# LimHaeryong/ESKF_LIO

Hardware: AMD Instinct MI355X
Metric: registered points/sec per VGICP iteration (100k-pt scan vs 1M-voxel map), 1/2/4/8 GPU (higher is better)
Workload: dtype f64

## Files before the change

### eskf_lio_amd/csrc/vgicp_kernels.hip

```cpp
#include <array>
#include <utility>

#include "vgicp_device.h"
#include "vgicp_device_fn.h"
#include "vgicp_launch_plan.h"
#include "vgicp_points_plan.h"

namespace vgicp {
namespace {

template <typename Args>
__device__ __forceinline__ bool scan_cov_symmetric(const Args& a) {
  return a.asym_dev != nullptr && *a.asym_dev != a.scan_seq;
}

template <int PIECES = 1>
__device__ __forceinline__ void unpack_payload(const double2* pay, double (&mu)[3], double (&S)[9]) {
  const double2 a0 = pay[0 * PIECES], a1 = pay[1 * PIECES], a2 = pay[2 * PIECES],
                a3 = pay[3 * PIECES], a4 = pay[4 * PIECES], a5 = pay[5 * PIECES];
  mu[0] = a0.x; mu[1] = a0.y; mu[2] = a1.x;
  S[0] = a1.y; S[1] = a2.x; S[2] = a2.y; S[3] = a3.x; S[4] = a3.y; S[5] = a4.x;
  S[6] = a4.y; S[7] = a5.x; S[8] = a5.y;
}
__device__ __forceinline__ void load_payload(const VoxelRecord* rec, double (&mu)[3], double (&S)[9]) {
// ... 836 lines not shown
  const int c_matched = __syncthreads_count(matched ? 1 : 0);
  const int c_counted = __syncthreads_count(counted ? 1 : 0);
  const int c_negative = __syncthreads_count(negative ? 1 : 0);
  const int c_not_finite = __syncthreads_count(not_finite ? 1 : 0);
  if (threadIdx.x == 0) {
    if (c_matched) atomicAdd(&a.counters[0], (uint32_t)c_matched);
    if (c_counted) atomicAdd(&a.counters[1], (uint32_t)c_counted);
    if (c_negative) atomicAdd(&a.counters[2], (uint32_t)c_negative);
    if (c_not_finite) atomicAdd(&a.counters[3], (uint32_t)c_not_finite);
  }
}

__global__ __launch_bounds__(256) void gate_decide_kernel(GateArgs a) {
  const uint32_t i = blockIdx.x * 256u + threadIdx.x;
  const bool cov_sym = scan_cov_symmetric(a);
  bool matched = false, refused = false, not_finite = false;
  if (i < a.n) {
    const PointTerm term = point_term(a, i, cov_sym);
    matched = term.matched;
    if (matched) {
      not_finite = !(fabs(term.raw) < __builtin_inf());
      refused = not_finite || !(fmax(term.raw, 0.0) <= a.gate);
    }
    a.keep[i] = refused ? (uint8_t)0 : (uint8_t)1;
  }
  const int c_matched = __syncthreads_count(matched ? 1 : 0);
  const int c_refused = __syncthreads_count(refused ? 1 : 0);
  const int c_not_finite = __syncthreads_count(not_finite ? 1 : 0);
  if (threadIdx.x == 0) {
    if (c_matched) atomicAdd(&a.counters[0], (uint32_t)c_matched);
    if (c_refused) atomicAdd(&a.counters[1], (uint32_t)c_refused);
    if (c_not_finite) atomicAdd(&a.counters[2], (uint32_t)c_not_finite);
  }
}

__global__ __launch_bounds__(64) void point_pick_kernel(PointPickArgs a) {
  const uint32_t lane = threadIdx.x;
  if (lane < (uint32_t)kPointCounters) a.out[lane] = a.counters[lane];
  if (lane < a.n_quantiles && lane < (uint32_t)kPointQuantiles) {
    const uint32_t matched = a.counters[0], not_finite = a.counters[3];
    const uint64_t m = matched > not_finite ? matched - not_finite : 0u;
    unsigned long long bits = 0x7FF8000000000000ull;
    if (m > 0) {
      const uint64_t rank = quantile_rank(a.q[lane], m);
      if (rank < a.n) bits = a.sorted[rank];
    }
    a.out[kPointCounters + lane] = bits;
  }
}

__global__ __launch_bounds__(64) void solve_step_kernel(const double* __restrict__ packed, double cos_thr,
                                                        double tsq_thr, int force_pivoted,
                                                        double* __restrict__ out) {
  __shared__ double totals[kSlots];
  __shared__ double work[kSolveWork];
  const uint32_t lane = threadIdx.x;
  if (lane < kSlots) totals[lane] = lane < kNormalEq ? packed[lane] : 0.0;
  __syncthreads();
  double A[21], g[6], xi[6];
#pragma unroll
  for (int k = 0; k < 21; ++k) A[k] = packed[k];
#pragma unroll
  for (int k = 0; k < 6; ++k) g[k] = -packed[21 + k];
  bool pivoted = force_pivoted != 0;
  if (pivoted || !ldlt6_solve_spd(A, g, xi)) {
    ldlt6_solve_pivoted(totals, work, lane, xi);
    pivoted = true;
  }
  Pose step;
  se3_exp_device(xi, step);
  const bool conv = converged(step, cos_thr, tsq_thr);
  if (lane == 0) {
#pragma unroll
    for (int k = 0; k < 6; ++k) out[k] = xi[k];
#pragma unroll
    for (int k = 0; k < 9; ++k) out[6 + k] = step.R[k];
#pragma unroll
    for (int k = 0; k < 3; ++k) out[15 + k] = step.t[k];
    out[18] = pivoted ? 1.0 : 0.0;
    out[19] = conv ? 1.0 : 0.0;
  }
}

typedef __attribute__((address_space(1))) unsigned long long gu64;
typedef __attribute__((address_space(1))) unsigned int gu32;

__device__ __forceinline__ void store_through_bits(double* p, unsigned long long bits) {
  __hip_atomic_store((gu64*)p, bits, __ATOMIC_RELAXED, __HIP_MEMORY_SCOPE_AGENT);
}
__device__ __forceinline__ unsigned long long load_through_bits(const double* p) {
  return __hip_atomic_load((gu64*)p, __ATOMIC_RELAXED, __HIP_MEMORY_SCOPE_AGENT);
}
__device__ __forceinline__ void store_system_bits(double* p, unsigned long long bits) {
  __hip_atomic_store((gu64*)p, bits, __ATOMIC_RELAXED, __HIP_MEMORY_SCOPE_SYSTEM);
}
__device__ __forceinline__ unsigned long long load_system_bits(const double* p) {
  return __hip_atomic_load((gu64*)p, __ATOMIC_RELAXED, __HIP_MEMORY_SCOPE_SYSTEM);
}
__device__ __forceinline__ unsigned long long publishable(double v) {
  const unsigned long long b = (unsigned long long)__double_as_longlong(v);
  return b == kRowUnset ? kRowNaN : b;
}

constexpr int kL2Delay = 64;
template <bool SYSTEM, bool LIVE = false>
__device__ __forceinline__ bool poll_and_sum(const double* src, uint32_t lane, uint32_t spin_limit, double& sum,
                                             uint32_t live = (uint32_t)kFolders) {
  constexpr int H = kFolders / 2;
  const uint32_t slot = lane & 31u, half = lane >> 5;
  const bool active = slot <= (uint32_t)kCountSlot;
  const double* mine = src + (size_t)half * H * kSlots + (active ? slot : 0u);
  unsigned long long w[H];
  if constexpr (LIVE) {
#pragma unroll
    for (int k = 0; k < H; ++k)
      w[k] = (active && half * H + (uint32_t)k < live) ? load_through_bits(mine + k * kSlots) : 0ull;
  } else {
#pragma unroll
    for (int k = 0; k < H; ++k)
      w[k] = active ? (SYSTEM ? load_system_bits(mine + k * kSlots) : load_through_bits(mine + k * kSlots)) : 0ull;
  }
  for (uint32_t spins = 0;; ++spins) {
    bool missing = false;
#pragma unroll
    for (int k = 0; k < H; ++k) missing = missing || (w[k] == kRowUnset);
    if (!__any(missing)) break;
    if (spins >= spin_limit) return false;
    __builtin_amdgcn_s_sleep(1);
#pragma unroll
    for (int k = 0; k < H; ++k)
      if (w[k] == kRowUnset) w[k] = SYSTEM ? load_system_bits(mine + k * kSlots) : load_through_bits(mine + k * kSlots);
  }
  double x[H];
#pragma unroll
  for (int k = 0; k < H; ++k) x[k] = __longlong_as_double((long long)w[k]);
  const double part = tree_sum<H>(x);
  const unsigned plo = (unsigned)__double2loint(part), phi = (unsigned)__double2hiint(part);
  const auto lo = __builtin_amdgcn_permlane32_swap(plo, plo, false, false);
  const auto hi = __builtin_amdgcn_permlane32_swap(phi, phi, false, false);
  sum = part + __hiloint2double((int)hi[1], (int)lo[1]);
  return true;
}

template <int N>
__device__ __forceinline__ uint64_t pinned_clock(double (&x)[N]) {
#pragma unroll
  for (int k = 0; k < N; ++k) asm volatile("" : "+v"(x[k]));
  const uint64_t t = wall_clock64();
#pragma unroll
  for (int k = 0; k < N; ++k) asm volatile("" : "+v"(x[k]));
  return t;
}

__device__ __forceinline__ bool fused_round0_load(const FusedUpload& f, uint64_t stride, uint32_t n_pts, double* lds,
                                                  double (&q0)[kScanPlanes]) {
  typedef int v4i __attribute__((ext_vector_type(4)));
  constexpr uint32_t B = 512, W = B - 64;
  __shared__ uint32_t ok_sh, form_sh[2];
  const uint32_t tid = threadIdx.x, p0 = blockIdx.x * W;
  const uint32_t cnt = p0 < n_pts ? min(W, n_pts - p0) : 0u;
  if (cnt == 0) return true;
  const uint32_t ua = p0 / f.unit, ub = (p0 + cnt - 1) / f.unit;
  const uint32_t split = min(p0 + cnt, (ua + 1) * f.unit);
  if (tid == 0) {
    uint32_t good = 1;
    for (uint32_t u = ua; u <= ub && good; ++u)
      for (uint32_t spins = 0; __hip_atomic_load(f.flags + 16 * u, __ATOMIC_RELAXED, __HIP_MEMORY_SCOPE_SYSTEM) != f.seq; ++spins) {
        if (spins >= f.spin_limit) { good = 0; break; }
        __builtin_amdgcn_s_sleep(20);
      }
    __atomic_thread_fence(__ATOMIC_ACQUIRE);
    ok_sh = good;
    if (good) {
      form_sh[0] = __hip_atomic_load(f.flags + 16 * ua + 1, __ATOMIC_RELAXED, __HIP_MEMORY_SCOPE_SYSTEM);
      form_sh[1] = __hip_atomic_load(f.flags + 16 * ub + 1, __ATOMIC_RELAXED, __HIP_MEMORY_SCOPE_SYSTEM);
    }
  }
  __syncthreads();
  if (!ok_sh) return false;
  double* lp = lds;
  double* lc = lds + 3 * W;
  double* lq = lds + 12 * W;
  {
    const v4i* sp = reinterpret_cast<const v4i*>(f.apts + (size_t)p0 * 24);
    const uint32_t np = (cnt * 24 + 15) / 16;
    for (uint32_t k = tid; k < np; k += B) reinterpret_cast<v4i*>(lp)[k] = __builtin_nontemporal_load(sp + k);
  }
  for (uint32_t s = 0; s < 2; ++s) {
    const uint32_t s0 = s ? split : p0, s1 = s ? p0 + cnt : split, u = s ? ub : ua;
    if (s0 >= s1) continue;
    if (form_sh[s] == kArenaCompact) {
      const v4i* sc = reinterpret_cast<const v4i*>(f.acov + (size_t)u * f.unit * 72 + (size_t)(s0 - u * f.unit) * 48);
      v4i* dst = reinterpret_cast<v4i*>(lq + 6 * (s0 - p0));
      for (uint32_t k = tid; k < (s1 - s0) * 3; k += B) dst[k] = __builtin_nontemporal_load(sc + k);
    } else {
      const v4i* sc = reinterpret_cast<const v4i*>(f.acov + (size_t)s0 * 72);
      v4i* dst = reinterpret_cast<v4i*>(lc + 9 * (s0 - p0));
      const uint32_t nc = ((s1 - s0) * 72 + 15) / 16;
      for (uint32_t k = tid; k < nc; k += B) dst[k] = __builtin_nontemporal_load(sc + k);
    }
  }
  __syncthreads();
  if (tid < cnt && form_sh[p0 + tid >= split ? 1 : 0] == kArenaCompact) {
    const double* q = lq + 6 * tid;
    const double a0 = q[0], a1 = q[1], a2 = q[2], a3 = q[3], a4 = q[4], a5 = q[5];
    double* c = lc + 9 * tid;
    c[0] = a0; c[1] = a1; c[2] = a2; c[3] = a1; c[4] = a3; c[5] = a4; c[6] = a2; c[7] = a4; c[8] = a5;
  }
  __syncthreads();
  if (tid == 0) atomicMax(f.unit_clock, (unsigned long long)wall_clock64());
  {
    const uint32_t wp = 3 * cnt, wc = 9 * cnt;
    v4i* dp = reinterpret_cast<v4i*>(f.aos_pts + 3 * (size_t)p0);
    v4i* dc = reinterpret_cast<v4i*>(f.aos_cov + 9 * (size_t)p0);
    for (uint32_t k = tid; k < wp / 2; k += B) dp[k] = reinterpret_cast<const v4i*>(lp)[k];
    for (uint32_t k = tid; k < wc / 2; k += B) dc[k] = reinterpret_cast<const v4i*>(lc)[k];
    if (tid == 0 && (cnt & 1u)) {
      f.aos_pts[3 * (size_t)p0 + wp - 1] = lp[wp - 1];
      f.aos_cov[9 * (size_t)p0 + wc - 1] = lc[wc - 1];
    }
  }
  const uint32_t wt = tid - 64u;
  if (tid >= 64u && wt < cnt) {
#pragma unroll
    for (int k = 0; k < 3; ++k) q0[k] = lp[3 * wt + k];
#pragma unroll
    for (int k = 0; k < 9; ++k) q0[3 + k] = lc[9 * wt + k];
    const size_t i = p0 + wt;
#pragma unroll
    for (int k = 0; k < kScanPlanes; ++k) f.soa[k * stride + i] = q0[k];
    const bool same = __double_as_longlong(q0[4]) == __double_as_longlong(q0[6]) &&
                      __double_as_longlong(q0[5]) == __double_as_longlong(q0[9]) &&
                      __double_as_longlong(q0[8]) == __double_as_longlong(q0[10]);
    if (!same) *f.asym = f.seq;
  }
  return true;
}

struct TeamView {
  uint32_t vb = 0;
  uint32_t team_wgs = 0;
  uint32_t folder_rows = 0;
  uint32_t* abort_word = nullptr;
};
template <int BLOCK, bool MULTI, bool STAMPS, bool MANY, bool FUSED = false, bool TEAM = false, bool ROBUST = false,
          bool PRIOR = false>
__device__ __forceinline__ void persistent_body(const PersistArgs& a, const FusedUpload& up, const TeamView& tv = TeamView()) {
  static_assert(!ROBUST || (!MULTI && !STAMPS && !FUSED && !TEAM), "the robust round runs the single-device bodies only");
  static_assert(!PRIOR || (!MULTI && !STAMPS && !FUSED && !TEAM), "the pose prior runs the single-device bodies only");
  static_assert(!FUSED || (!MULTI && !STAMPS && !MANY), "the fused upload serves the single-device one-point-per-thread body");
  static_assert(!TEAM || (!MULTI && !STAMPS && !MANY && !FUSED), "teams run the single-device one-point-per-thread body");
  static_assert(BLOCK / kSlots == kFolders, "the exchange reproduces the fold order of iterate_kernel<512>");
  constexpr int kWaves = BLOCK / 64;
  constexpr int kWorkers = BLOCK - 64;
  __shared__ double red[kWaves][kSlots];
  __shared__ double totals[kSlots];
  __shared__ double work[kSolveWork];
  __shared__ double pose_sh[12];
  __shared__ int stop_sh;
  extern __shared__ __attribute__((aligned(16))) unsigned char dyn_lds[];
  int4* pf_key = reinterpret_cast<int4*>(dyn_lds);
  double2* pf_pay = reinterpret_cast<double2*>(dyn_lds + (size_t)kWorkers * sizeof(int4));
  const bool prefetch = !MANY && a.prefetch_margin > 0.0;

  const uint32_t tid = threadIdx.x, lane = tid & 63, wave = tid >> 6;
  const uint32_t n_pts = a.n_dev ? (*a.n_dev < a.n ? *a.n_dev : a.n) : a.n;
  const bool cov_sym = MANY && scan_cov_symmetric(a);
  const uint32_t grid = gridDim.x, blk = TEAM ? tv.vb : blockIdx.x;
  constexpr uint32_t W = MANY ? (uint32_t)BLOCK : (uint32_t)kWorkers;
  const bool worker = MANY || wave != 0;
  const uint32_t wt = MANY ? tid : tid - 64u;
  uint32_t stride_pts = grid * W, first = worker ? blk * W + wt : n_pts, end_pts = n_pts;
  if constexpr (MANY) {
    const uint32_t units = (n_pts + 63u) / 64u, share = units / grid, extra = units % grid;
    const uint32_t u0 = blk * share + (blk < extra ? blk : extra), u1 = u0 + share + (blk < extra ? 1u : 0u);
    stride_pts = W;
    first = u0 * 64u + wt;
    end_pts = u1 * 64u < n_pts ? u1 * 64u : n_pts;
  }
  const VoxelRecord* pay_base = a.dense ? a.dense : a.table;
  int4* memo = reinterpret_cast<int4*>(dyn_lds);
  double* stash = reinterpret_cast<double*>(dyn_lds + (size_t)a.memo_points * W * sizeof(int4));
  const uint32_t park_planes = cov_sym ? 9u : (uint32_t)kScanPlanes;
  const uint32_t fit = a.stash_bytes / (park_planes * W * (uint32_t)sizeof(double));
  const uint32_t parked = MANY ? (fit < a.stash_points ? fit : a.stash_points) : 0u;
  const bool folder = blk < (uint32_t)kFolders;
  const uint32_t my_row = TEAM ? (blk % kFolders) * tv.folder_rows + blk / kFolders : (blk % kFolders) * kFolders + blk / kFolders;
  const uint32_t buf_rows = TEAM ? (uint32_t)kFolders * tv.folder_rows : (uint32_t)kExchangeRows;
  const uint32_t live_rows = TEAM ? (tv.team_wgs - blk + (uint32_t)kFolders - 1u) / (uint32_t)kFolders : (uint32_t)kFolders;
  const uint32_t live_parts = TEAM ? (tv.team_wgs < (uint32_t)kFolders ? tv.team_wgs : (uint32_t)kFolders) : (uint32_t)kFolders;

  Pose total;
#pragma unroll
  for (int k = 0; k < 9; ++k) total.R[k] = a.pose0[k];
#pragma unroll
  for (int k = 0; k < 3; ++k) total.t[k] = a.pose0[9 + k];
  const double cos_thr = a.cosine_threshold, tsq_thr = a.translation_sq_threshold;
  const int max_it = a.max_iteration;
  const double inv_voxel = 1.0 / a.voxel_size;
  const double same_margin = 0x1p-20 * a.voxel_size;
  RobustSetting robust;
  if constexpr (ROBUST) robust = robust_setting(a.robust.kernel, a.robust.scale2, a.robust.gate);

  double q0[kScanPlanes];
#pragma unroll
  for (int k = 0; k < kScanPlanes; ++k) q0[k] = 0.0;
  const bool have = first < end_pts;
  if constexpr (FUSED) {
    if (!fused_round0_load(up, a.stride, n_pts, reinterpret_cast<double*>(dyn_lds), q0)) {
      if (tid == 0) a.state->abort_seq = a.seq;
      return;
    }
  } else if (have) {
    load_point(a.scan, a.stride, first, q0);
  }

  bool spec = false, hit = false;
  int32_t okx = 0, oky = 0, okz = 0;
  double mu[3] = {0.0, 0.0, 0.0}, Sv[9];
#pragma unroll
  for (int k = 0; k < 9; ++k) Sv[k] = 0.0;

  uint64_t t_mark = STAMPS ? wall_clock64() : 0;
  uint64_t acc_body = 0, acc_l1 = 0, acc_l2 = 0, acc_solve = 0;
  uint64_t fine[4] = {0, 0, 0, 0};
  bool conv_keep = false;
  int it = 0;
  bool gave_up = false;
  for (;;) {
    const double* R = total.R;
    const double* t = total.t;
    if (worker) {
      double v[kSlots];
#pragma unroll
      for (int k = 0; k < kSlots; ++k) v[k] = 0.0;
      if constexpr (!MANY) {
        if (have) {
          double p[3], C[9], S[9];
#pragma unroll
          for (int k = 0; k < 9; ++k) C[k] = q0[3 + k];
          transform_point(R, t, q0[0], q0[1], q0[2], p);
          const int32_t kx = voxel_coord_fast(p[0], a.voxel_size, inv_voxel);
          const int32_t ky = voxel_coord_fast(p[1], a.voxel_size, inv_voxel);
          const int32_t kz = voxel_coord_fast(p[2], a.voxel_size, inv_voxel);
          if (!spec || kx != okx || ky != oky || kz != okz) {
            bool served = false;
            if (spec && prefetch) {
              const int4 m = pf_key[tid - 64];
              if (m.x == kx && m.y == ky && m.z == kz && (uint32_t)m.w != kMemoNone) {
                served = true;
                hit = (uint32_t)m.w != kMemoMiss;
                if (hit) unpack_payload<kWorkers>(pf_pay + (tid - 64), mu, Sv);
              }
            }
            if (!served) hit = find_and_load(a.table, a.mask, kx, ky, kz, mu, Sv);
            okx = kx; oky = ky; okz = kz;
            spec = true;
          }
          if (hit) {
#pragma unroll
            for (int k = 0; k < 9; ++k) S[k] = Sv[k];
            accumulate_match<true, ROBUST>(R, p, C, mu, S, v, robust);
          }
        }
      } else {
        auto one_point = [&](const double (&q)[kScanPlanes], uint32_t e, auto first_of_round) {
          double p[3], C[9], m2[3], S[9];
          transform_point(R, t, q[0], q[1], q[2], p);
          bool got;
          if (e < a.memo_points) {
            int4* mslot = memo + (size_t)e * W + wt;
            const int4 m = *mslot;
            const bool stayed = ((int)(it != 0) & (int)same_voxel_coord(p[0], m.x, a.voxel_size, same_margin) &
                                 (int)same_voxel_coord(p[1], m.y, a.voxel_size, same_margin) &
                                 (int)same_voxel_coord(p[2], m.z, a.voxel_size, same_margin)) != 0;
            if (stayed) {
              got = (uint32_t)m.w != kMemoMiss;
              if (got) load_payload(pay_base + (uint32_t)m.w, m2, S);
            } else {
              const int32_t kx = voxel_coord_fast(p[0], a.voxel_size, inv_voxel);
              const int32_t ky = voxel_coord_fast(p[1], a.voxel_size, inv_voxel);
              const int32_t kz = voxel_coord_fast(p[2], a.voxel_size, inv_voxel);
              if (it != 0 && m.x == kx && m.y == ky && m.z == kz) {
                got = (uint32_t)m.w != kMemoMiss;
                if (got) load_payload(pay_base + (uint32_t)m.w, m2, S);
              } else {
                const VoxelRecord* rec = find_voxel(a.table, a.mask, kx, ky, kz);
                got = rec != nullptr;
                uint32_t where = kMemoMiss;
                if (got) where = a.dense ? reinterpret_cast<const uint32_t*>(&rec->reserved)[1] : (uint32_t)(rec - a.table);
                *mslot = make_int4(kx, ky, kz, (int32_t)where);
                if (got) load_payload(rec, m2, S);
              }
            }
          } else {
            const int32_t kx = voxel_coord_fast(p[0], a.voxel_size, inv_voxel);
            const int32_t ky = voxel_coord_fast(p[1], a.voxel_size, inv_voxel);
            const int32_t kz = voxel_coord_fast(p[2], a.voxel_size, inv_voxel);
            got = find_and_load(a.table, a.mask, kx, ky, kz, m2, S);
          }
          if (got) {
#pragma unroll
            for (int k = 0; k < 9; ++k) C[k] = q[3 + k];
            accumulate_match<decltype(first_of_round)::value, ROBUST>(R, p, C, m2, S, v, robust);
          }
        };
        if (have) one_point(q0, 0u, Flag<true>{});
        uint32_t e = 1;
        for (uint32_t i = first + stride_pts; i < end_pts; i += stride_pts, ++e) {
          double q[kScanPlanes];
          if (e <= parked) {
            double* slot = stash + (size_t)(e - 1) * park_planes * W + wt;
            if (it == 0) {
              load_point_sym(a.scan, a.stride, i, q, cov_sym);
              if (cov_sym) {
                constexpr int kUsed[9] = {0, 1, 2, 3, 4, 5, 7, 8, 11};
#pragma unroll
                for (int j = 0; j < 9; ++j) slot[j * W] = q[kUsed[j]];
              } else {
#pragma unroll
                for (int k = 0; k < kScanPlanes; ++k) slot[k * W] = q[k];
              }
            } else if (cov_sym) {
              constexpr int kUsed[9] = {0, 1, 2, 3, 4, 5, 7, 8, 11};
#pragma unroll
              for (int j = 0; j < 9; ++j) q[kUsed[j]] = slot[j * W];
              q[6] = q[4]; q[9] = q[5]; q[10] = q[8];
            } else {
#pragma unroll
              for (int k = 0; k < kScanPlanes; ++k) q[k] = slot[k * W];
            }
          } else {
            load_point_sym(a.scan, a.stride, i, q, cov_sym);
          }
          one_point(q, e, Flag<false>{});
        }
      }
      wave_fold_to_lds(v, lane, red[wave]);
    }
    __syncthreads();
    if (STAMPS) { const uint64_t n = wall_clock64(); acc_body += n - t_mark; t_mark = n; }

    if (!MANY && worker && prefetch && have) {
      double p[3], rx, ry, rz;
      transform_point(R, t, q0[0], q0[1], q0[2], p);
      (void)voxel_coord_fast(p[0], a.voxel_size, inv_voxel, &rx);
      (void)voxel_coord_fast(p[1], a.voxel_size, inv_voxel, &ry);
      (void)voxel_coord_fast(p[2], a.voxel_size, inv_voxel, &rz);
      const double half = 0.5 * a.voxel_size;
      const double dx = fmin(rx, a.voxel_size - rx), dy = fmin(ry, a.voxel_size - ry), dz = fmin(rz, a.voxel_size - rz);
      int32_t nx = okx, ny = oky, nz = okz;
      double d;
      if (dx <= dy && dx <= dz) { d = dx; nx += rx < half ? -1 : 1; }
      else if (dy <= dz) { d = dy; ny += ry < half ? -1 : 1; }
      else { d = dz; nz += rz < half ? -1 : 1; }
      int4 m = make_int4(nx, ny, nz, (int32_t)kMemoNone);
      if (d < a.prefetch_margin * a.voxel_size) {
        const VoxelRecord* rec = find_voxel(a.table, a.mask, nx, ny, nz);
        m.w = rec ? (int32_t)(uint32_t)(rec - a.table) : (int32_t)kMemoMiss;
        if (rec) {
          const double2* pay = reinterpret_cast<const double2*>(rec->mean);
          double2* dst = pf_pay + (tid - 64);
#pragma unroll
          for (int j = 0; j < 6; ++j) dst[j * kWorkers] = pay[j];
        }
      }
      pf_key[tid - 64] = m;
    }
    if (STAMPS && !MANY && wave != 0) { asm volatile("s_waitcnt vmcnt(0) lgkmcnt(0)" ::: "memory"); const uint64_t n = wall_clock64(); acc_l1 += n - t_mark; t_mark = n; }

    if (wave == 0) {
      uint32_t lane_here = tid & 63;
      asm volatile("" : "+v"(lane_here));
      const uint32_t lane = lane_here;
      const uint32_t buf = (a.round0 + (uint32_t)it) % 3u;
      double* rows = a.rows + (size_t)buf * buf_rows * kSlots;
      double* parts = a.parts + (size_t)buf * kFolders * kSlots;
      asm volatile("s_waitcnt vmcnt(0)" ::: "memory");
      if (lane <= (uint32_t)kCountSlot) {
        double w_sum[kWaves];
#pragma unroll
        for (int w = 0; w < kWaves; ++w) w_sum[w] = red[w][lane];
        const double row_sum = MANY ? tree_sum<kWaves>(w_sum) : tree_sum<kWaves - 1>(w_sum + 1);
        store_through_bits(rows + (size_t)my_row * kSlots + lane, publishable(row_sum));
      }
      bool ok = true;
      const uint32_t spin_limit = (FUSED && it == 0 && up.spin_limit > a.spin_limit) ? up.spin_limit : a.spin_limit;
      if (folder) {
        double part = 0.0;
        if constexpr (TEAM) ok = poll_and_sum<false, true>(rows + (size_t)blk * tv.folder_rows * kSlots, lane, spin_limit, part, live_rows);
        else ok = poll_and_sum<false>(rows + (size_t)blk * kFolders * kSlots, lane, spin_limit, part);
        if (ok && lane <= (uint32_t)kCountSlot) store_through_bits(parts + (size_t)blk * kSlots + lane, publishable(part));
      }
      if (STAMPS) { const uint64_t n = wall_clock64(); acc_l1 += n - t_mark; t_mark = n; }
      double tot = 0.0;
      if (!MULTI) {
        if (!MANY && !folder) __builtin_amdgcn_s_sleep(kL2Delay);
        if constexpr (TEAM) { if (ok) ok = poll_and_sum<false, true>(parts, lane, spin_limit, tot, live_parts); }
        else if (ok) ok = poll_and_sum<false>(parts, lane, spin_limit, tot);
      } else {
        const uint32_t mbuf = (a.mail_round0 + (uint32_t)it) % 3u;
        if (blk == 0) {
          double mine = 0.0;
          if (ok) ok = poll_and_sum<false>(parts, lane, a.spin_limit, mine);
          if (ok && lane <= (uint32_t)kCountSlot) {
            const unsigned long long bits = publishable(mine);
            for (uint32_t r = 0; r < a.world; ++r)
              store_system_bits(a.mail[r] + ((size_t)mbuf * kMaxRanks + a.rank) * kSlots + lane, bits);
          }
        }
        if (ok) ok = poll_and_sum<true>(a.mail[a.rank] + (size_t)mbuf * kMaxRanks * kSlots, lane, a.spin_limit, tot);
      }
      if (STAMPS) { const uint64_t n = wall_clock64(); acc_l2 += n - t_mark; t_mark = n; }
      if (!ok) {
        if (lane == 0) stop_sh = 2;
      } else {
        if (lane < kSlots) totals[lane] = lane <= (uint32_t)kCountSlot ? tot : 0.0;
        __builtin_amdgcn_fence(__ATOMIC_RELEASE, "wavefront");
        __builtin_amdgcn_wave_barrier();
        __builtin_amdgcn_fence(__ATOMIC_ACQUIRE, "wavefront");
        const double* solve = totals;
        if constexpr (PRIOR) solve = prior_solve_totals(a, total, totals, lane);
        double A[21], g[6], xi[6];
#pragma unroll
        for (int k = 0; k < 21; ++k) A[k] = solve[k];
#pragma unroll
        for (int k = 0; k < 6; ++k) g[k] = -solve[21 + k];
        uint64_t f0 = 0, f1 = 0, f2 = 0;
        if (STAMPS) { f0 = pinned_clock(A); fine[0] += f0 - t_mark; }
        if (!ldlt6_solve_spd(A, g, xi)) ldlt6_solve_pivoted(solve, work, lane, xi);
        if (STAMPS) { f1 = pinned_clock(xi); fine[1] += f1 - f0; }
        Pose next, step;
        se3_exp_device(xi, step);
        pose_compose(step, total, next);
        conv_keep = converged(step, cos_thr, tsq_thr);
        if (STAMPS) { f2 = pinned_clock(next.R); fine[2] += f2 - f1; }
        if (lane == 0) {
#pragma unroll
          for (int k = 0; k < 9; ++k) pose_sh[k] = next.R[k];
#pragma unroll
          for (int k = 0; k < 3; ++k) pose_sh[9 + k] = next.t[k];
          stop_sh = (conv_keep || (it + 1 >= max_it)) ? 1 : 0;
        }
        if (STAMPS) fine[3] += wall_clock64() - f2;
      }
    }
    __syncthreads();
    const int stop = stop_sh;
    if (stop == 2) { gave_up = true; break; }
    if (wave == 0) {
      uint32_t lane_here = tid & 63;
      asm volatile("" : "+v"(lane_here));
      const uint32_t rearm = (a.round0 + (uint32_t)it + 2u) % 3u;
      if (lane_here <= (uint32_t)kCountSlot) {
        store_through_bits(a.rows + ((size_t)rearm * buf_rows + my_row) * kSlots + lane_here, kRowUnset);
        if (folder) store_through_bits(a.parts + ((size_t)rearm * kFolders + blk) * kSlots + lane_here, kRowUnset);
      }
      if (MULTI && blk == 0 && lane_here <= (uint32_t)kCountSlot) {
        const uint32_t old = (a.mail_round0 + (uint32_t)it + 2u) % 3u;
        for (uint32_t r = 0; r < a.world; ++r)
          store_system_bits(a.mail[a.rank] + ((size_t)old * kMaxRanks + r) * kSlots + lane_here, kRowUnset);
      }
      if (blk == 0 && lane_here < kSlots) a.log[(size_t)it * kSlots + lane_here] = totals[lane_here];
    }
    load_pose(pose_sh, total);
    ++it;
    if (STAMPS) { const uint64_t n = wall_clock64(); acc_solve += n - t_mark; t_mark = n; }
    if (stop) break;
  }
  if (gave_up) {
    if (tid == 0) { if constexpr (TEAM) *tv.abort_word = a.seq; else a.state->abort_seq = a.seq; }
    if (MULTI && blk == 0 && tid < a.world)
      store_system_bits(a.mail[tid] + kMailRowWords + a.rank, (unsigned long long)a.mail_seq << 1);
    return;
  }

  if (wave == 0 && blk == 0) {
    uint32_t outcome = kOutcomeCommitted;
    if (MULTI) {
      const unsigned long long mine = ((unsigned long long)a.mail_seq << 1) | 1ull;
      if (lane < a.world) store_system_bits(a.mail[lane] + kMailRowWords + a.rank, mine);
      const double* src = a.mail[a.rank] + kMailRowWords + (lane < a.world ? lane : 0u);
      unsigned long long w = lane < a.world ? load_system_bits(src) : mine;
      bool late = false;
      for (uint32_t spins = 0; __any((w >> 1) < a.mail_seq); ++spins) {
        if (spins >= a.spin_limit) { late = true; break; }
        __builtin_amdgcn_s_sleep(1);
        if ((w >> 1) < a.mail_seq) w = load_system_bits(src);
      }
      if (late) outcome = kOutcomeNoAgreement;
      else if (__any(w != mine)) outcome = kOutcomeAgreedAbort;
    }
    if (lane == 0) {
      AlignState* out = a.state;
      out->outcome = outcome;
      if (outcome == kOutcomeCommitted) {
#pragma unroll
        for (int k = 0; k < 9; ++k) out->pose[k] = total.R[k];
#pragma unroll
        for (int k = 0; k < 3; ++k) out->pose[9 + k] = total.t[k];
        out->cosine_threshold = cos_thr;
        out->translation_sq_threshold = tsq_thr;
        out->max_iteration = max_it;
        out->iteration = it;
        out->converged = conv_keep ? 1 : 0;
        out->done = 1;
        out->pad = 0;
        if constexpr (FUSED)
          out->unit_to_end_ticks = wall_clock64() - __hip_atomic_load(up.unit_clock, __ATOMIC_RELAXED, __HIP_MEMORY_SCOPE_AGENT);
        out->seq = a.seq;
      }
    }
  }
  if (STAMPS && tid == 0) atomicAdd((unsigned long long*)&a.stamps[32 + blk], (unsigned long long)acc_body);
  if (STAMPS && blk == 0 && (tid == 0 || tid == 64)) {
    const int o = tid == 0 ? 8 : 16;
    atomicAdd((unsigned long long*)&a.stamps[o + 0], (unsigned long long)acc_body);
    atomicAdd((unsigned long long*)&a.stamps[o + 1], (unsigned long long)acc_l1);
    atomicAdd((unsigned long long*)&a.stamps[o + 2], (unsigned long long)acc_l2);
    atomicAdd((unsigned long long*)&a.stamps[o + 3], (unsigned long long)acc_solve);
    atomicAdd((unsigned long long*)&a.stamps[o + 5], (unsigned long long)it);
    if (tid == 0)
      for (int k = 0; k < 4; ++k) atomicAdd((unsigned long long*)&a.stamps[24 + k], (unsigned long long)fine[k]);
  }
}

template <int BLOCK, bool MULTI, bool STAMPS, bool MANY, bool ROBUST = false, bool PRIOR = false>
__global__ __launch_bounds__(BLOCK) void persistent_kernel(PersistArgs a) {
  const FusedUpload none{};
  if constexpr (MANY) {
    const uint32_t n_pts = a.n_dev ? (*a.n_dev < a.n ? *a.n_dev : a.n) : a.n;
    if (n_pts <= gridDim.x * (uint32_t)(BLOCK - 64)) {
      persistent_body<BLOCK, MULTI, STAMPS, false, false, false, ROBUST, PRIOR>(a, none);
      return;
    }
  }
  persistent_body<BLOCK, MULTI, STAMPS, MANY, false, false, ROBUST, PRIOR>(a, none);
}

template <int BLOCK>
__global__ __launch_bounds__(BLOCK) void persistent_fused_kernel(PersistArgs a, FusedUpload up) {
  persistent_body<BLOCK, false, false, false, true>(a, up);
}

template <int BLOCK>
__global__ __launch_bounds__(BLOCK) void persistent_team_kernel(PersistArgs a, TeamArgs t) {
  const uint32_t h = blockIdx.x / t.team_wgs;
  if (h >= t.teams) return;
  const FusedUpload none{};
  TeamView tv;
  tv.vb = blockIdx.x - h * t.team_wgs;
  tv.team_wgs = t.team_wgs;
  tv.folder_rows = t.folder_rows;
  tv.abort_word = t.abort_word;
  a.rows += (size_t)h * 3 * kFolders * t.folder_rows * kSlots;
  a.parts += (size_t)h * 3 * kFolders * kSlots;
  a.state = reinterpret_cast<AlignState*>(reinterpret_cast<double*>(a.state) + (size_t)h * t.slot_words);
  a.log += (size_t)h * t.slot_words;
#pragma unroll
  for (int k = 0; k < 12; ++k) a.pose0[k] = t.pose0[h][k];
  persistent_body<BLOCK, false, false, false, false, true>(a, none, tv);
}

__global__ __launch_bounds__(1024) void fold_rows_kernel(const double* __restrict__ rows,
                                                         uint32_t nrows, const AlignState* state,
                                                         double* __restrict__ sums) {
  constexpr int kGroups = 1024 / kSlots;
  __shared__ double fin[kGroups][kSlots];
  if (state->done) return;
  const uint32_t tid = threadIdx.x, slot = tid & (kSlots - 1), group = tid / kSlots;
  double s = 0.0;
  for (uint32_t b = group; b < nrows; b += kGroups) s += rows[(size_t)b * kSlots + slot];
  fin[group][slot] = s;
  __syncthreads();
  if (tid < kSlots) {
    double tot = fin[0][tid];
#pragma unroll
    for (int g = 1; g < kGroups; ++g) tot += fin[g][tid];
    sums[tid] = tot;
  }
}

__global__ void gather_scan_kernel(const uint32_t* __restrict__ perm, uint32_t m, const double* __restrict__ pts,
                                   const double* __restrict__ covs, const unsigned long long* __restrict__ idx,
                                   double* __restrict__ out_pts, double* __restrict__ out_covs,
                                   unsigned long long* __restrict__ out_idx) {
  const uint32_t o = blockIdx.x * blockDim.x + threadIdx.x;
  if (o >= m) return;
  const uint32_t from = perm[o];
#pragma unroll
  for (int k = 0; k < 3; ++k) out_pts[3 * (size_t)o + k] = pts[3 * (size_t)from + k];
#pragma unroll
  for (int k = 0; k < 9; ++k) out_covs[9 * (size_t)o + k] = covs[9 * (size_t)from + k];
  if (idx) out_idx[o] = idx[from];
}

__global__ void pack_scan_kernel(const double* __restrict__ pts, const double* __restrict__ covs,
                                 uint32_t n, double* __restrict__ soa, uint64_t stride, uint32_t* asym, uint32_t seq) {
  const uint32_t i = blockIdx.x * blockDim.x + threadIdx.x;
  if (i >= n) return;
#pragma unroll
  for (int k = 0; k < 3; ++k) soa[k * stride + i] = pts[3 * (size_t)i + k];
  double c[9];
#pragma unroll
  for (int k = 0; k < 9; ++k) {
    c[k] = covs[9 * (size_t)i + k];
    soa[(3 + k) * stride + i] = c[k];
  }
  const bool same = __double_as_longlong(c[1]) == __double_as_longlong(c[3]) &&
                    __double_as_longlong(c[2]) == __double_as_longlong(c[6]) &&
                    __double_as_longlong(c[5]) == __double_as_longlong(c[7]);
  if (!same) *asym = seq;
}

constexpr int kPackArenaBlock = 256;
__global__ __launch_bounds__(kPackArenaBlock) void pack_arena_kernel(
    const char* __restrict__ apts, const char* __restrict__ acov, uint32_t n, uint32_t unit, const uint32_t* flags,
    uint32_t wait, uint32_t seq, uint32_t spin_limit, double* __restrict__ aos_pts, double* __restrict__ aos_cov,
    double* __restrict__ soa, uint64_t stride, uint32_t* asym) {
  typedef int v4i __attribute__((ext_vector_type(4)));
  constexpr uint32_t B = kPackArenaBlock;
  __shared__ __attribute__((aligned(16))) double lds[12 * B];
  __shared__ __attribute__((aligned(16))) double lds_compact[6 * B];
  __shared__ uint32_t ok, form_sh;
  const uint32_t t = threadIdx.x, blocks = (n + B - 1) / B;
  uint32_t have_unit = 0xFFFFFFFFu;
  for (uint32_t b = blockIdx.x; b < blocks; b += gridDim.x) {
    const uint32_t p0 = b * B, cnt = min(B, n - p0);
    const uint32_t u = p0 / unit;
    if (u != have_unit) {
      if (t == 0) {
        uint32_t good = 1;
        if (wait)
          for (uint32_t spins = 0; __hip_atomic_load(flags + 16 * u, __ATOMIC_RELAXED, __HIP_MEMORY_SCOPE_SYSTEM) != seq; ++spins) {
            if (spins >= spin_limit) { good = 0; break; }
            __builtin_amdgcn_s_sleep(20);
          }
        __atomic_thread_fence(__ATOMIC_ACQUIRE);
        ok = good;
        form_sh = good ? __hip_atomic_load(flags + 16 * u + 1, __ATOMIC_RELAXED, __HIP_MEMORY_SCOPE_SYSTEM) : kArenaFull;
      }
      __syncthreads();
      if (!ok) return;
      have_unit = u;
    }
    const bool compact = form_sh == kArenaCompact;
    const v4i* sp = reinterpret_cast<const v4i*>(apts + (size_t)p0 * 24);
    v4i* lp = reinterpret_cast<v4i*>(lds);
    v4i* lc = reinterpret_cast<v4i*>(lds + 3 * B);
    const uint32_t np = (cnt * 24 + 15) / 16, np_whole = (cnt * 24) / 16, nc = (cnt * 72 + 15) / 16, nc_whole = (cnt * 72) / 16;
    v4i* dp = reinterpret_cast<v4i*>(aos_pts + 3 * (size_t)p0);
    v4i* dc = reinterpret_cast<v4i*>(aos_cov + 9 * (size_t)p0);
    for (uint32_t k = t; k < np; k += B) {
      const v4i w = __builtin_nontemporal_load(sp + k);
      lp[k] = w;
      if (k < np_whole) dp[k] = w;
    }
    if (!compact) {
      const v4i* sc = reinterpret_cast<const v4i*>(acov + (size_t)p0 * 72);
      for (uint32_t k = t; k < nc; k += B) {
        const v4i w = __builtin_nontemporal_load(sc + k);
        lc[k] = w;
        if (k < nc_whole) dc[k] = w;
      }
    } else {
      const uint32_t u0 = u * unit;
      const v4i* sc = reinterpret_cast<const v4i*>(acov + (size_t)u0 * 72 + (size_t)(p0 - u0) * 48);
      v4i* lq = reinterpret_cast<v4i*>(lds_compact);
      for (uint32_t k = t; k < cnt * 3; k += B) lq[k] = __builtin_nontemporal_load(sc + k);
    }
    __syncthreads();
    if (t == 0 && np != np_whole) {
      aos_pts[3 * (size_t)(p0 + cnt) - 1] = lds[3 * cnt - 1];
      if (!compact) aos_cov[9 * (size_t)(p0 + cnt) - 1] = lds[3 * B + 9 * cnt - 1];
    }
    if (t < cnt) {
      const size_t i = p0 + t;
#pragma unroll
      for (int k = 0; k < 3; ++k) soa[k * stride + i] = lds[3 * t + k];
      double c[9];
      if (compact) {
        const double a0 = lds_compact[6 * t], a1 = lds_compact[6 * t + 1], a2 = lds_compact[6 * t + 2],
                     a3 = lds_compact[6 * t + 3], a4 = lds_compact[6 * t + 4], a5 = lds_compact[6 * t + 5];
        c[0] = a0; c[1] = a1; c[2] = a2; c[3] = a1; c[4] = a3; c[5] = a4; c[6] = a2; c[7] = a4; c[8] = a5;
#pragma unroll
        for (int k = 0; k < 9; ++k) lds[3 * B + 9 * t + k] = c[k];
      } else {
#pragma unroll
        for (int k = 0; k < 9; ++k) c[k] = lds[3 * B + 9 * t + k];
      }
#pragma unroll
      for (int k = 0; k < 9; ++k) soa[(3 + k) * stride + i] = c[k];
      const bool same = __double_as_longlong(c[1]) == __double_as_longlong(c[3]) &&
                        __double_as_longlong(c[2]) == __double_as_longlong(c[6]) &&
                        __double_as_longlong(c[5]) == __double_as_longlong(c[7]);
      if (!same) *asym = seq;
    }
    __syncthreads();
    if (compact) {
      const uint32_t words = cnt * 9;
      for (uint32_t k = t; k < words / 2; k += B) dc[k] = lc[k];
      if (t == 0 && (words & 1u)) aos_cov[9 * (size_t)p0 + words - 1] = lds[3 * B + words - 1];
      __syncthreads();
    }
  }
}

}

namespace {
using IterateFn = void (*)(IterArgs);
using PersistentFn = void (*)(PersistArgs);
template <size_t... I>
constexpr std::array<IterateFn, sizeof...(I)> iterate_table(std::index_sequence<I...>) {
  return {{&iterate_kernel<kIterateVariants[I].block, kIterateVariants[I].robust, kIterateVariants[I].prior>...}};
}
template <size_t... I>
constexpr std::array<IterateFn, sizeof...(I)> close_table(std::index_sequence<I...>) {
  return {{&close_kernel<kCloseVariants[I].block, kCloseVariants[I].prior>...}};
}
template <size_t... I>
constexpr std::array<PersistentFn, sizeof...(I)> persistent_table(std::index_sequence<I...>) {
  return {{&persistent_kernel<512, kPersistentVariants[I].multi, kPersistentVariants[I].stamps, kPersistentVariants[I].many,
                              kPersistentVariants[I].robust, kPersistentVariants[I].prior>...}};
}
constexpr auto kIterateKernels = iterate_table(std::make_index_sequence<kIterateVariantCount>{});
constexpr auto kCloseKernels = close_table(std::make_index_sequence<kCloseVariantCount>{});
constexpr auto kPersistentKernels = persistent_table(std::make_index_sequence<kPersistentVariantCount>{});
}

hipError_t launch_iterate(hipStream_t s, const IterArgs& args, uint32_t grid, int block) {
  const int v = plan_iterate(block, args.robust.kernel, args.robust.gate, args.prior.on != 0);
  if (v == kLaunchRefused) return hipErrorInvalidValue;
  counted_launch(kIterateKernels[v], dim3(grid), dim3(block), 0, s, args);
  return hipGetLastError();
}

namespace {
static_assert(kMemoBytesPerPoint == kPersistWide * sizeof(int4) &&
              kPrefetchBytes == kPersistWorkers * (sizeof(int4) + 6 * sizeof(double2)), "the plan's LDS sizes are the kernel's");
constexpr uint32_t kMaxMemoPoints = 12;
constexpr uint32_t kFusedLoadBytes = kPersistWorkers * 18 * sizeof(double);
}

void persistent_lds_plan(uint32_t n, uint32_t grid, uint32_t* memo_points, uint32_t* stash_points, uint32_t* stash_bytes,
                         uint32_t lds_budget) {
  *memo_points = *stash_points = *stash_bytes = 0;
  const uint32_t budget = (lds_budget == 0 || lds_budget > kPersistDynLds) ? kPersistDynLds : lds_budget;
  if ((uint64_t)n <= (uint64_t)grid * kPersistWorkers) return;
  const uint32_t units = (n + 63u) / 64u, most = (units + grid - 1) / grid;
  const uint32_t per_thread = (most + kPersistWide / 64 - 1) / (kPersistWide / 64);
  uint32_t memo = per_thread < kMaxMemoPoints ? per_thread : kMaxMemoPoints;
  if (memo * kMemoBytesPerPoint > budget) memo = budget / kMemoBytesPerPoint;
  *memo_points = memo;
  *stash_points = per_thread - 1;
  *stash_bytes = *stash_points ? budget - memo * kMemoBytesPerPoint : 0u;
}

size_t persistent_rows_words() { return 3 * (size_t)kExchangeRows * kSlots; }
size_t persistent_parts_words() { return 3 * (size_t)kFolders * kSlots; }

void persistent_exchange_image(uint32_t grid, unsigned long long* rows_words, unsigned long long* parts_words) {
  for (int buf = 0; buf < 3; ++buf) {
    unsigned long long* rw = rows_words + (size_t)buf * kExchangeRows * kSlots;
    for (size_t w = 0; w < (size_t)kExchangeRows * kSlots; ++w) rw[w] = 0ull;
    for (uint32_t b = 0; b < grid && b < (uint32_t)kExchangeRows; ++b) {
      const uint32_t row = (b % kFolders) * kFolders + b / kFolders;
      for (int sl = 0; sl <= kCountSlot; ++sl) rw[(size_t)row * kSlots + sl] = kRowUnset;
    }
    unsigned long long* pw = parts_words + (size_t)buf * kFolders * kSlots;
    for (size_t w = 0; w < (size_t)kFolders * kSlots; ++w) pw[w] = 0ull;
    for (uint32_t g = 0; g < grid && g < (uint32_t)kFolders; ++g)
      for (int sl = 0; sl <= kCountSlot; ++sl) pw[(size_t)g * kSlots + sl] = kRowUnset;
  }
}

hipError_t persistent_prepare_device() {
  hipError_t e = hipFuncSetAttribute(reinterpret_cast<const void*>(&persistent_fused_kernel<512>),
                                     hipFuncAttributeMaxDynamicSharedMemorySize, (int)kPersistDynLds);
  for (PersistentFn fn : kPersistentKernels)
    if (e == hipSuccess)
      e = hipFuncSetAttribute(reinterpret_cast<const void*>(fn), hipFuncAttributeMaxDynamicSharedMemorySize, (int)kPersistDynLds);
  return e;
}

hipError_t launch_persistent(hipStream_t s, const PersistArgs& args, uint32_t grid) {
  PersistentFacts f;
  f.world = args.world;
  f.stamps = args.stamps != nullptr;
  f.n = args.n;
  f.grid = grid;
  f.memo_points = args.memo_points;
  f.stash_bytes = args.stash_bytes;
// ... 133 lines not shown
```

Before: 5.960 billion.

## Defer fused upload write-back past first iteration and skip redundant prefetch lookups

```diff
diff --git a/eskf_lio_amd/csrc/vgicp_kernels.hip b/eskf_lio_amd/csrc/vgicp_kernels.hip
--- a/eskf_lio_amd/csrc/vgicp_kernels.hip
+++ b/eskf_lio_amd/csrc/vgicp_kernels.hip
@@ -1012,29 +1012,52 @@
   return t;
 }
 
+__device__ __forceinline__ unsigned long long load_flag_and_form(const uint32_t* flags, uint32_t u) {
+  return __hip_atomic_load((gu64*)(flags + 16 * (size_t)u), __ATOMIC_RELAXED, __HIP_MEMORY_SCOPE_SYSTEM);
+}
+
+struct FusedLeave {
+  double* plane;
+  double* aos_pts;
+  double* aos_cov;
+  uint32_t* asym;
+  uint64_t stride;
+  uint32_t seq, cnt;
+};
+
 __device__ __forceinline__ bool fused_round0_load(const FusedUpload& f, uint64_t stride, uint32_t n_pts, double* lds,
-                                                  double (&q0)[kScanPlanes]) {
+                                                  FusedLeave* leave, double (&q0)[kScanPlanes]) {
   typedef int v4i __attribute__((ext_vector_type(4)));
   constexpr uint32_t B = 512, W = B - 64;
   __shared__ uint32_t ok_sh, form_sh[2];
   const uint32_t tid = threadIdx.x, p0 = blockIdx.x * W;
   const uint32_t cnt = p0 < n_pts ? min(W, n_pts - p0) : 0u;
+  if (tid == 0) {
+    leave->plane = f.soa + p0;
+    leave->aos_pts = f.aos_pts + 3 * (size_t)p0;
+    leave->aos_cov = f.aos_cov + 9 * (size_t)p0;
+    leave->asym = f.asym;
+    leave->stride = stride;
+    leave->seq = f.seq;
+    leave->cnt = cnt;
+  }
   if (cnt == 0) return true;
   const uint32_t ua = p0 / f.unit, ub = (p0 + cnt - 1) / f.unit;
   const uint32_t split = min(p0 + cnt, (ua + 1) * f.unit);
   if (tid == 0) {
     uint32_t good = 1;
-    for (uint32_t u = ua; u <= ub && good; ++u)
-      for (uint32_t spins = 0; __hip_atomic_load(f.flags + 16 * u, __ATOMIC_RELAXED, __HIP_MEMORY_SCOPE_SYSTEM) != f.seq; ++spins) {
+    for (uint32_t u = ua; u <= ub && good; ++u) {
+      unsigned long long w = load_flag_and_form(f.flags, u);
+      for (uint32_t spins = 0; (uint32_t)w != f.seq; ++spins) {
         if (spins >= f.spin_limit) { good = 0; break; }
         __builtin_amdgcn_s_sleep(20);
+        w = load_flag_and_form(f.flags, u);
       }
+      form_sh[u == ua ? 0 : 1] = (uint32_t)(w >> 32);
+    }
+    if (ua == ub) form_sh[1] = form_sh[0];
     __atomic_thread_fence(__ATOMIC_ACQUIRE);
     ok_sh = good;
-    if (good) {
-      form_sh[0] = __hip_atomic_load(f.flags + 16 * ua + 1, __ATOMIC_RELAXED, __HIP_MEMORY_SCOPE_SYSTEM);
-      form_sh[1] = __hip_atomic_load(f.flags + 16 * ub + 1, __ATOMIC_RELAXED, __HIP_MEMORY_SCOPE_SYSTEM);
-    }
   }
   __syncthreads();
   if (!ok_sh) return false;
@@ -1069,32 +1092,39 @@
   }
   __syncthreads();
   if (tid == 0) atomicMax(f.unit_clock, (unsigned long long)wall_clock64());
-  {
-    const uint32_t wp = 3 * cnt, wc = 9 * cnt;
-    v4i* dp = reinterpret_cast<v4i*>(f.aos_pts + 3 * (size_t)p0);
-    v4i* dc = reinterpret_cast<v4i*>(f.aos_cov + 9 * (size_t)p0);
-    for (uint32_t k = tid; k < wp / 2; k += B) dp[k] = reinterpret_cast<const v4i*>(lp)[k];
-    for (uint32_t k = tid; k < wc / 2; k += B) dc[k] = reinterpret_cast<const v4i*>(lc)[k];
-    if (tid == 0 && (cnt & 1u)) {
-      f.aos_pts[3 * (size_t)p0 + wp - 1] = lp[wp - 1];
-      f.aos_cov[9 * (size_t)p0 + wc - 1] = lc[wc - 1];
-    }
-  }
   const uint32_t wt = tid - 64u;
   if (tid >= 64u && wt < cnt) {
 #pragma unroll
     for (int k = 0; k < 3; ++k) q0[k] = lp[3 * wt + k];
 #pragma unroll
     for (int k = 0; k < 9; ++k) q0[3 + k] = lc[9 * wt + k];
-    const size_t i = p0 + wt;
-#pragma unroll
-    for (int k = 0; k < kScanPlanes; ++k) f.soa[k * stride + i] = q0[k];
+  }
+  return true;
+}
+
+__device__ __forceinline__ void fused_leave_resident(const FusedLeave* leave, const double* lds, const double (&q0)[kScanPlanes]) {
+  constexpr uint32_t W = 512 - 64;
+  uint32_t tid_here = threadIdx.x;
+  asm volatile("" : "+v"(tid_here));
+  const uint32_t wt = tid_here - 64u;
+  const FusedLeave to = *leave;
+  const double* lp = lds;
+  const double* lc = lds + 3 * W;
+  if (wt < to.cnt) {
+    double* plane = to.plane + wt;
+#pragma unroll 1
+    for (int k = 0; k < 3; ++k, plane += to.stride) store_through_bits(plane, (unsigned long long)__double_as_longlong(lp[3 * wt + k]));
+#pragma unroll 1
+    for (int k = 0; k < 9; ++k, plane += to.stride) store_through_bits(plane, (unsigned long long)__double_as_longlong(lc[9 * wt + k]));
     const bool same = __double_as_longlong(q0[4]) == __double_as_longlong(q0[6]) &&
                       __double_as_longlong(q0[5]) == __double_as_longlong(q0[9]) &&
                       __double_as_longlong(q0[8]) == __double_as_longlong(q0[10]);
-    if (!same) *f.asym = f.seq;
-  }
-  return true;
+    if (!same) *to.asym = to.seq;
+  }
+#pragma unroll 1
+  for (uint32_t k = wt; k < 3 * to.cnt; k += W) store_through_bits(to.aos_pts + k, (unsigned long long)__double_as_longlong(lp[k]));
+#pragma unroll 1
+  for (uint32_t k = wt; k < 9 * to.cnt; k += W) store_through_bits(to.aos_cov + k, (unsigned long long)__double_as_longlong(lc[k]));
 }
 
 struct TeamView {
@@ -1118,6 +1148,7 @@
   __shared__ double work[kSolveWork];
   __shared__ double pose_sh[12];
   __shared__ int stop_sh;
+  __shared__ FusedLeave leave_sh;
   extern __shared__ __attribute__((aligned(16))) unsigned char dyn_lds[];
   int4* pf_key = reinterpret_cast<int4*>(dyn_lds);
   double2* pf_pay = reinterpret_cast<double2*>(dyn_lds + (size_t)kWorkers * sizeof(int4));
@@ -1167,13 +1198,15 @@
   for (int k = 0; k < kScanPlanes; ++k) q0[k] = 0.0;
   const bool have = first < end_pts;
   if constexpr (FUSED) {
-    if (!fused_round0_load(up, a.stride, n_pts, reinterpret_cast<double*>(dyn_lds), q0)) {
+    if (!fused_round0_load(up, a.stride, n_pts, reinterpret_cast<double*>(dyn_lds), &leave_sh, q0)) {
       if (tid == 0) a.state->abort_seq = a.seq;
       return;
     }
   } else if (have) {
     load_point(a.scan, a.stride, first, q0);
   }
+
+  constexpr int kFirstLook = FUSED ? 1 : 0;
 
   bool spec = false, hit = false;
   int32_t okx = 0, oky = 0, okz = 0;
@@ -1205,7 +1238,7 @@
           const int32_t kz = voxel_coord_fast(p[2], a.voxel_size, inv_voxel);
           if (!spec || kx != okx || ky != oky || kz != okz) {
             bool served = false;
-            if (spec && prefetch) {
+            if (spec && prefetch && it > kFirstLook) {
               const int4 m = pf_key[tid - 64];
               if (m.x == kx && m.y == ky && m.z == kz && (uint32_t)m.w != kMemoNone) {
                 served = true;
@@ -1301,7 +1334,9 @@
     __syncthreads();
     if (STAMPS) { const uint64_t n = wall_clock64(); acc_body += n - t_mark; t_mark = n; }
 
-    if (!MANY && worker && prefetch && have) {
+    if (FUSED && it == 0) {
+      if (worker) fused_leave_resident(&leave_sh, reinterpret_cast<const double*>(dyn_lds), q0);
+    } else if (!MANY && worker && prefetch && have) {
       double p[3], rx, ry, rz;
       transform_point(R, t, q0[0], q0[1], q0[2], p);
       (void)voxel_coord_fast(p[0], a.voxel_size, inv_voxel, &rx);
@@ -1314,18 +1349,21 @@
       if (dx <= dy && dx <= dz) { d = dx; nx += rx < half ? -1 : 1; }
       else if (dy <= dz) { d = dy; ny += ry < half ? -1 : 1; }
       else { d = dz; nz += rz < half ? -1 : 1; }
-      int4 m = make_int4(nx, ny, nz, (int32_t)kMemoNone);
-      if (d < a.prefetch_margin * a.voxel_size) {
-        const VoxelRecord* rec = find_voxel(a.table, a.mask, nx, ny, nz);
-        m.w = rec ? (int32_t)(uint32_t)(rec - a.table) : (int32_t)kMemoMiss;
-        if (rec) {
-          const double2* pay = reinterpret_cast<const double2*>(rec->mean);
-          double2* dst = pf_pay + (tid - 64);
-#pragma unroll
-          for (int j = 0; j < 6; ++j) dst[j * kWorkers] = pay[j];
+      const int4 known = pf_key[tid - 64];
+      if (it == kFirstLook || known.x != nx || known.y != ny || known.z != nz || (uint32_t)known.w == kMemoNone) {
+        int4 m = make_int4(nx, ny, nz, (int32_t)kMemoNone);
+        if (d < a.prefetch_margin * a.voxel_size) {
+          const VoxelRecord* rec = find_voxel(a.table, a.mask, nx, ny, nz);
+          m.w = rec ? (int32_t)(uint32_t)(rec - a.table) : (int32_t)kMemoMiss;
+          if (rec) {
+            const double2* pay = reinterpret_cast<const double2*>(rec->mean);
+            double2* dst = pf_pay + (tid - 64);
+#pragma unroll
+            for (int j = 0; j < 6; ++j) dst[j * kWorkers] = pay[j];
+          }
         }
+        pf_key[tid - 64] = m;
       }
-      pf_key[tid - 64] = m;
     }
     if (STAMPS && !MANY && wave != 0) { asm volatile("s_waitcnt vmcnt(0) lgkmcnt(0)" ::: "memory"); const uint64_t n = wall_clock64(); acc_l1 += n - t_mark; t_mark = n; }
 
@@ -1591,14 +1629,16 @@
     if (u != have_unit) {
       if (t == 0) {
         uint32_t good = 1;
+        unsigned long long w = load_flag_and_form(flags, u);
         if (wait)
-          for (uint32_t spins = 0; __hip_atomic_load(flags + 16 * u, __ATOMIC_RELAXED, __HIP_MEMORY_SCOPE_SYSTEM) != seq; ++spins) {
+          for (uint32_t spins = 0; (uint32_t)w != seq; ++spins) {
             if (spins >= spin_limit) { good = 0; break; }
             __builtin_amdgcn_s_sleep(20);
+            w = load_flag_and_form(flags, u);
           }
         __atomic_thread_fence(__ATOMIC_ACQUIRE);
         ok = good;
-        form_sh = good ? __hip_atomic_load(flags + 16 * u + 1, __ATOMIC_RELAXED, __HIP_MEMORY_SCOPE_SYSTEM) : kArenaFull;
+        form_sh = good ? (uint32_t)(w >> 32) : kArenaFull;
       }
       __syncthreads();
       if (!ok) return;
```

Result: faster. 6.407 billion (median of 6 runs) (+7.5%).
